# pd3/bcftools

Measured on AMD Instinct MI355X. Metric: variant sites/sec (mpileup|call -m), 1000-sample 30x WGS synthetic, higher is better.
Workload: dtype u8/i32 + f64 likelihood sums

## Files before the change

### bcftools_amd/csrc/api.hip

```cpp
#include <hip/hip_runtime.h>
#include <cstdio>
#include <cstdlib>
#include <cstring>
#include <cmath>
#include <string>
#include <vector>
#include <algorithm>
#include "ctx.h"
#include "tables.h"

using namespace bcfgpu;

static thread_local std::string g_err;
static int set_err(int code, const char *what, hipError_t e = hipSuccess)
{
    char buf[512];
    if (e != hipSuccess) snprintf(buf, sizeof buf, "%s: %s", what, hipGetErrorString(e));
    else snprintf(buf, sizeof buf, "%s", what);
    g_err = buf;
    return code;
}
#define HIPCHK(call) do { hipError_t e_ = (call); if (e_ != hipSuccess) return set_err(BCFGPU_E_HIP, #call, e_); } while (0)

struct bcfgpu_ctx {
// ... 338 lines not shown
    if (!c) return BCFGPU_E_ARG;
    c->timing = on;
    if (on == 2) while (c->pool.size() < 4 * 64) { hipEvent_t e; hipEventCreate(&e); c->pool.push_back(e); }
    return 0;
}
int bcfgpu_timing_get(bcfgpu_ctx *c, bcfgpu_timing *t)
{
    if (!c || !t) return set_err(BCFGPU_E_ARG, "bcfgpu_timing_get: bad arguments");
    if (c->timing == 2) {
        bcfgpu_timing a{};
        const size_t n = c->pool_call.size();
        if (n) {
            HIPCHK(hipStreamSynchronize(c->stream));
            int ncall = 0;
            for (size_t k = 0; k < n; ++k) {
                hipEvent_t *e = &c->pool[4 * k];
                float g = 0, m = 0, q = 0, tot = 0;
                hipEventElapsedTime(&g, e[0], e[1]);
                hipEventElapsedTime(&m, e[1], e[2]);
                if (c->pool_call[k]) { hipEventElapsedTime(&q, e[2], e[3]); hipEventElapsedTime(&tot, e[0], e[3]); ncall++; }
                else hipEventElapsedTime(&tot, e[0], e[2]);
                a.glfgen_ms += g; a.combine_ms += m; a.mcall_ms += q; a.total_ms += tot;
            }
            a.glfgen_ms /= n; a.combine_ms /= n; a.total_ms /= n;
            if (ncall) a.mcall_ms /= ncall;
            c->pool_used = 0; c->pool_call.clear();
        }
        c->last = a;
    }
    *t = c->last;
    return 0;
}

static hipEvent_t *seq_events(bcfgpu_ctx *c)
{
    if (c->timing == 2) {
        while (c->pool.size() < c->pool_used + 4) { hipEvent_t e; hipEventCreate(&e); c->pool.push_back(e); }
        c->pool_call.push_back(0);
        c->pool_used += 4;
        return &c->pool[c->pool_used - 4];
    }
    return c->ev;
}

static int check_tile(bcfgpu_ctx *c, const bcfgpu_tile *t)
{
    if (!t || t->n_sites < 0) return set_err(BCFGPU_E_ARG, "bad tile");
    if (t->n_sites > c->cfg.max_sites || t->n_reads > c->cfg.max_reads)
        return set_err(BCFGPU_E_RANGE, "tile exceeds the capacity the context was created with");
    if (t->n_sites && (!t->plp_off || (!t->is_indel && !t->ref16) || (t->n_reads && (!t->rd || !t->epos))))
        return set_err(BCFGPU_E_ARG, "tile: NULL array");
    if (t->is_indel && t->n_reads && !t->aux) return set_err(BCFGPU_E_ARG, "indel tile without aux");
    if (((uintptr_t)t->rd & 15) || ((uintptr_t)t->epos & 15) || (t->is_indel && ((uintptr_t)t->aux & 15)))
        return set_err(BCFGPU_E_ARG, "tile: rd/epos/aux must be 16-byte aligned");
    if (t->n_reads >> 32) return set_err(BCFGPU_E_RANGE, "tile: more than 2^32-1 reads");
    return 0;
}

static int enqueue_mpileup(bcfgpu_ctx *c, const bcfgpu_tile *tile, const bcfgpu_mplp_out *out)
{
    const int S = c->cfg.n_smpl;
    GlfgenParams g{};
    g.n_sites = tile->n_sites; g.n_smpl = S; g.is_indel = tile->is_indel;
    g.min_baseQ = c->cfg.min_baseQ; g.capQ = c->cfg.capQ; g.fmt_flag = c->cfg.fmt_flag;
    const int slots = 255 / S + 2;
    g.hist_slots = slots <= 8 ? slots : 0;
    {
        const double mean = (double)tile->n_reads / ((double)tile->n_sites * S);
        long want = (long)(mean * 256 * 1.03) + 64;
        want = std::max(2048L, (want + 15) & ~15L);
        int cap = 0;
        for (int wgs = 6; wgs >= 3 && !cap; --wgs) {
            const long budget = (long)(128 / wgs) * 1280 - 32;
            long c = (budget - (long)glfgen_lds_bytes(0, g.hist_slots)) / 2;
            c = std::min(c & ~15L, (long)GLF_MAX_WINDOW);
            if (c >= want || wgs == 3) cap = (int)std::max(c, 2048L);
        }
        g.lds_cap = cap;
        int pc = 64;
        while (pc > 4 && 17 * std::max(g.hist_slots, 1) * pc > 2048) pc >>= 1;
        g.part_cols = pc;
    }
    g.n_reads = (uint32_t)tile->n_reads;
    g.ref16 = tile->ref16; g.off = tile->plp_off; g.rd = tile->rd; g.epos = tile->epos; g.aux = tile->aux;
    g.fk = c->d_fk; g.beta = c->d_beta; g.lhet = c->d_lhet; g.pfx = c->d_pfx;
    g.crp = c->d_crp;
    g.hist = c->d_hist; g.err = c->d_err; g.site_sums = c->d_site_sums;
    g.trunc = reinterpret_cast<unsigned int*>(c->d_err + 1);
    g.deep_list = c->d_deep_list; g.deep_ctr = reinterpret_cast<uint32_t*>(c->d_err + 2); g.deep_keys = c->d_deep_keys;
    g.deep_cap = c->deep_cap; g.deep_key_cap = c->deep_key_cap;
    {
        const int kind = tile->is_indel ? 1 : 0;
        g.draw_bits = (c->draw.rd[kind] && c->draw.rd[kind] == tile->rd && c->draw.n_reads[kind] == tile->n_reads) ? c->draw.bits[kind] : nullptr;
        c->draw.rd[kind] = nullptr;
    }
    g.wide_ctr = reinterpret_cast<uint32_t*>(c->d_err + 5); g.wide_cap = c->wide_cap;
    HIPCHK(hipMemsetAsync(c->d_err + 2, 0, 4 * sizeof(int), c->stream));
    HIPCHK(hipMemsetAsync(c->d_hist, 0, (size_t)tile->n_sites * H_SIZE * sizeof(int), c->stream));
    HIPCHK(hipMemsetAsync(c->d_site_sums, 0, (size_t)tile->n_sites * SITE_NSUM * 8, c->stream));
    hipEvent_t *ev = c->timing ? seq_events(c) : nullptr;
    if (ev) hipEventRecord(ev[0], c->stream);
    launch_glfgen(g, c->stream);
    if (ev) hipEventRecord(ev[1], c->stream);
    CombineParams k{};
    k.n_sites = tile->n_sites; k.n_smpl = S; k.is_indel = tile->is_indel; k.fmt_flag = c->cfg.fmt_flag;
    k.ref16 = tile->ref16; k.cr = c->cr; k.hist = c->d_hist; k.site_sums = c->d_site_sums; k.mw = c->d_mw; k.out = *out;
    launch_combine(k, c->stream);
    if (ev) hipEventRecord(ev[2], c->stream);
    HIPCHK(hipGetLastError());
    return 0;
}

static void finish_timing(bcfgpu_ctx *c, bool with_call)
{
    if (c->timing != 1) return;
    hipEventSynchronize(with_call ? c->ev[3] : c->ev[2]);
    bcfgpu_timing t{};
    hipEventElapsedTime(&t.glfgen_ms, c->ev[0], c->ev[1]);
    hipEventElapsedTime(&t.combine_ms, c->ev[1], c->ev[2]);
    if (with_call) hipEventElapsedTime(&t.mcall_ms, c->ev[2], c->ev[3]);
    hipEventElapsedTime(&t.total_ms, c->ev[0], with_call ? c->ev[3] : c->ev[2]);
    c->last = t;
}

int bcfgpu_mpileup(bcfgpu_ctx *c, const bcfgpu_tile *tile, const bcfgpu_mplp_out *out)
{
    if (!c || !out || !out->site || !out->pl || !out->dp4) return set_err(BCFGPU_E_ARG, "bcfgpu_mpileup: bad arguments");
    int rc = check_tile(c, tile);
    if (rc) return rc;
    if (tile->n_sites == 0) return 0;
    hipSetDevice(c->cfg.device);
    rc = enqueue_mpileup(c, tile, out);
    if (rc) return rc;
    finish_timing(c, false);
    return 0;
}

static float *grp_q_for(bcfgpu_ctx *c, int n_sites)
{
    if (c->cfg.n_grp <= 1 || n_sites <= 0) return nullptr;
    const size_t bytes = (size_t)n_sites * c->cfg.n_grp * 5 * sizeof(float);
    if (bytes <= c->grp_q_bytes) return c->d_grp_q;
    if (c->d_grp_q) { hipStreamSynchronize(c->stream); hipFree(c->d_grp_q); c->d_grp_q = nullptr; c->grp_q_bytes = 0; }
    void *p = nullptr;
    if (hipMalloc(&p, bytes + bytes / 4) != hipSuccess) { (void)hipGetLastError(); return nullptr; }
    c->d_grp_q = (float*)p; c->grp_q_bytes = bytes + bytes / 4;
    return c->d_grp_q;
}

int bcfgpu_mcall(bcfgpu_ctx *c, const bcfgpu_call_in *in, const bcfgpu_call_out *out)
{
    if (!c || !in || !out || !out->site || !out->gt) return set_err(BCFGPU_E_ARG, "bcfgpu_mcall: bad arguments");
    if (in->n_sites == 0) return 0;
    if (!in->nals || !in->unseen || !in->pl || (!in->qs && !(c->cfg.n_grp > 1)))
        return set_err(BCFGPU_E_ARG, "bcfgpu_mcall: NULL input array");
    if (c->cfg.n_grp > 1 && (!in->grp || !in->ad)) return set_err(BCFGPU_E_ARG, "bcfgpu_mcall: -G needs grp and ad");
    if (in->n_gt_max < 1 || in->n_gt_max > BCFGPU_MAX_PL) return set_err(BCFGPU_E_ARG, "bcfgpu_mcall: n_gt_max out of range");
    if (in->ad && (in->n_al_max < 1 || in->n_al_max > BCFGPU_MAX_ALLELES)) return set_err(BCFGPU_E_ARG, "bcfgpu_mcall: n_al_max out of range");
    hipSetDevice(c->cfg.device);
    McallParams m{};
    m.n_sites = in->n_sites; m.n_smpl = c->cfg.n_smpl; m.n_gt_max = in->n_gt_max; m.n_al_max = in->n_al_max;
    m.pl_is_u8 = 0; m.call_flag = c->cfg.call_flag; m.output_tags = c->cfg.output_tags; m.n_grp = c->cfg.n_grp;
    m.theta = c->call_theta_log; m.pl2p = c->d_pl2p;
    m.nals = in->nals; m.unseen = in->unseen; m.msite = nullptr; m.pl = in->pl; m.qs = in->qs; m.ad = in->ad;
    m.grp_rng = c->d_grp_rng; m.grp_q = grp_q_for(c, m.n_sites);
    if (c->cfg.n_grp > 1 && !m.grp_q) return set_err(BCFGPU_E_NOMEM, "call -G: workspace of the groups' frequency sums");
// ... 143 lines not shown
```

### bcftools_amd/csrc/glfgen.hip

```cpp
#include <hip/hip_runtime.h>
#include <cstdlib>
#include "kernels.h"

namespace bcfgpu {

#define WG 256
#ifndef GLF_WAVES
#define GLF_WAVES 5
#endif
#define DEF_MAPQ 20
#define CAP_DIST 25

#define NT16_INT_TBL 0x4444444344424104ull
__device__ __forceinline__ int nt16_int(int c) { return (int)((NT16_INT_TBL >> (4 * (c & 15))) & 7); }
__device__ __forceinline__ int tri(int j, int k) { return k * (k + 1) / 2 + j; }

__device__ __forceinline__ uint32_t wave_sum_u32(uint32_t v)
{
    #pragma unroll
    for (int o = 32; o > 0; o >>= 1) v += __shfl_xor(v, o);
    return v;
}

#define LDS_FK   0
#define LDS_CNT  2112
#ifndef NRANK
#define NRANK 10
#endif
#define NSLOT    NRANK
#ifndef FU
#define FU       4
#endif
#define LDS_HIST_OFF (LDS_CNT + NSLOT * WG * 4)
#define HP_SIZE 280
#define HP_MQS  220
#define HP_MAX  0xffffu
static_assert(GLF_MAX_WINDOW <= HP_MAX, "one round's window alone must fit a 16-bit half of the packed histograms");
static_assert(H_SIZE <= 2 * HP_SIZE, "a deep cell's 32-bit histograms take the LDS of two packed slots (hist_slots >= 2 whenever it is not 0)");
#define NPART 17
static_assert(NPART == SITE_NSUM + 3, "phase A's partial sums: the site totals and three mapQ >= 59 counts");

#define KEY_PACK(rev, q, b, sc) ((uint32_t)(rev) | (uint32_t)(q) << 1 | (uint32_t)(b) << 7 | (uint32_t)(sc) << 10)
#define KEY_REV(k)  ((k) & 1u)
#define KEY_Q(k)    (((k) >> 1) & 63u)
#define KEY_B(k)    (((k) >> 7) & 7u)
#define KEY_SC(k)   (((k) >> 10) & 1u)
#define KEY_PRIM    0x800u

#ifndef WR
#define WR 2
#endif
struct PrimSrc {
    const uint16_t *kpp;
    __device__ __forceinline__ uint32_t key(int j) const { return kpp[j]; }
    __device__ __forceinline__ bool ok(uint32_t k) const { return k != 0; }
    __device__ __forceinline__ int operator()(int j) const { const uint32_t k = key(j); return ok(k) ? (int)(k & 0x7f) : -1; }
};
struct BaseSrc {
    const uint16_t *kp; int b;
    __device__ __forceinline__ uint32_t key(int i) const { return kp[i]; }
    __device__ __forceinline__ bool ok(uint32_t k) const { return KEY_B(k) == (uint32_t)b; }
    __device__ __forceinline__ int operator()(int i) const { const uint32_t k = key(i); return ok(k) ? (int)(k & 0x7f) : -1; }
};
__device__ __forceinline__ uint32_t popc64(uint64_t x) { return (uint32_t)__popc((uint32_t)x) + (uint32_t)__popc((uint32_t)(x >> 32)); }
template <bool FIRST, bool CHK, class Src>
__device__ __forceinline__ void count_keys(uint32_t *s_slot, uint64_t qm, int tid, Src src, int nsrc)
{
    const uint64_t qm1 = qm >> 1;
    for (int j = 0; __any(j < nsrc); j += FU) {
        if (j < nsrc) {
            uint32_t k4[FU];
            #pragma unroll
            for (int u = 0; u < FU; ++u) k4[u] = src.key(j + u);
            #pragma unroll
            for (int u = 0; u < FU; ++u) {
                const uint32_t k = k4[u], q = KEY_Q(k);
                const uint32_t r = popc64(qm1 >> q);
                bool take = src.ok(k) && (u == 0 || j + u < nsrc);
                if (!FIRST) take = take && ((qm >> q) & 1ull);
                if (CHK) take = take && r < (uint32_t)NRANK;
                const uint32_t rv = (uint32_t)((int32_t)(k << 31) >> 31);
                if (take) atomicAdd(&s_slot[r * WG + tid], (rv & 1u) | (~rv & 0x100u));
            }
        }
    }
}
template <bool FIRST, class Src>
__device__ __forceinline__ uint32_t count_runs(uint32_t *s_slot, uint64_t qm, int tid, Src src, int nsrc)
{
    #pragma unroll
    for (int k = 0; k < NRANK; ++k) s_slot[k * WG + tid] = 0;
    if (__any(popc64(qm) > (uint32_t)NRANK)) count_keys<FIRST, true>(s_slot, qm, tid, src, nsrc);
    else count_keys<FIRST, false>(s_slot, qm, tid, src, nsrc);
    uint32_t qs = 0;
    uint64_t m = qm;
    #pragma unroll
    for (int r = 0; r < NRANK && __any(m != 0); ++r) {
        if (m != 0) {
            const uint32_t q = 63u - (uint32_t)__builtin_clzll(m);
            const uint32_t c = s_slot[r * WG + tid];
            s_slot[r * WG + tid] = c | q << 16;
            qs = __builtin_amdgcn_udot4(c, q | q << 8, qs, false);
            m &= ~(1ull << q);
        }
    }
    return qs;
}

template <class Src>
__device__ __forceinline__ double walk_runs(uint32_t *s_slot, uint64_t qm, const double *s_fk, const char *bbase, const double *pfx, int tid,
                                            uint32_t brow, Src src, int nsrc, uint32_t &rev_out, uint32_t &qs_out)
{
    double bs = 0;
    uint32_t qs = 0;
    uint32_t wpack = 0;
    uint32_t cnt = 0;
    uint32_t koff = brow;
    uint32_t qoff = 0;
    uint32_t r = 0;
    uint32_t d_nx = 0;
    auto slot_of = [&](uint32_t rk) -> uint32_t { return s_slot[min(rk, (uint32_t)NRANK - 1u) * WG + tid]; };
    auto step = [&](uint32_t (&off)[WR], uint32_t (&wi)[WR]) -> bool {
        const bool pop = cnt == 0 && r < NRANK;
        cnt = pop ? (d_nx & 0xffu) | (d_nx & 0xff00u) << 8 : cnt;
        qoff = pop ? (d_nx & 0x3f0000u) << 3 : qoff;
        r += pop ? 1u : 0u;
        d_nx = slot_of(r);
        const uint32_t sh = (cnt & 0xffffu) ? 0u : 16u;
        const uint32_t left = (cnt >> sh) & 0xffffu;
        const uint32_t w = (wpack >> sh) & 0xffffu;
        const uint32_t o1 = qoff + koff;
        #pragma unroll
        for (uint32_t u = 0; u < WR; ++u) {
            const bool act = left > u;
            wi[u] = act ? w + u : 256u;
            off[u] = act ? o1 + (u << 11) : brow;
        }
        const uint32_t took = min(left, (uint32_t)WR);
        wpack += took << sh; cnt -= took << sh;
        koff += took << 11;
        return __any(left != 0);
    };
    #define WALK_LOAD(B, F, off_, wi_) do { _Pragma("unroll") for (int u_ = 0; u_ < WR; ++u_) { \
        B[u_] = *reinterpret_cast<const double*>(bbase + (off_)[u_]); F[u_] = s_fk[(wi_)[u_]]; } } while (0)
    #define WALK_ADD(B, F) do { _Pragma("unroll") for (int u_ = 0; u_ < WR; ++u_) bs += F[u_] * B[u_]; } while (0)
    bool first = true;
    while (__any(qm != 0)) {
        qs += first ? count_runs<true>(s_slot, qm, tid, src, nsrc) : count_runs<false>(s_slot, qm, tid, src, nsrc);
        r = 0;
        d_nx = slot_of(0);
        const uint32_t d0 = d_nx, r1 = d0 & 0xffu, f1 = (d0 >> 8) & 0xffu;
        const bool tb = first && brow < (uint32_t)GLF_PFX_N << 3 && (d0 & 0xe0e0u) == 0u && (d0 & 0xffffu) != 0u;
        const uint32_t ti = tb ? (d0 & 0x3f0000u) | brow << 7 | r1 << 5 | f1 : 0u;
        const double t0 = pfx[ti];
        wpack = tb ? r1 | f1 << 16 : wpack;
        koff = tb ? brow + ((r1 + f1) << 11) : koff;
        r = tb ? 1u : 0u;
        d_nx = slot_of(r);
        first = false;
        double bx[WR], fx[WR], by[WR], fy[WR];
        uint32_t off[WR], wi[WR];
        bool ax = step(off, wi);
        WALK_LOAD(bx, fx, off, wi);
        bool ay = step(off, wi);
        WALK_LOAD(by, fy, off, wi);
        bs = tb ? t0 : bs;
        while (ax) {
            WALK_ADD(bx, fx);
            ax = step(off, wi);
            WALK_LOAD(bx, fx, off, wi);
            if (!ay) break;
            WALK_ADD(by, fy);
            ay = step(off, wi);
            WALK_LOAD(by, fy, off, wi);
        }
        WALK_ADD(bx, fx);
        WALK_ADD(by, fy);
        if (__any(__popcll(qm) > NRANK)) {
            uint64_t m = qm;
            for (int k = 0; k < NRANK && m; ++k) m &= ~(1ull << (63 - __clzll((long long)m)));
            qm = m;
        } else qm = 0;
    }
    #undef WALK_ADD
    #undef WALK_LOAD
    rev_out = wpack & 0xffffu; qs_out = qs;
    return bs;
}

struct ReadSums {
    uint32_t t_bq, t_bq2, t_mq, t_mq2, t_md, t_md2;
    uint32_t d_bq, d_bq2, d_mq, d_mq2, d_md, d_md2;
    __device__ __forceinline__ void clear() { t_bq = t_bq2 = t_mq = t_mq2 = t_md = t_md2 = d_bq = d_bq2 = d_mq = d_mq2 = d_md = d_md2 = 0; }
};
struct ReadCounts {
    uint32_t ori, mq0, m59, ref59, rev59;
    __device__ __forceinline__ void clear() { ori = mq0 = m59 = ref59 = rev59 = 0; }
};
typedef unsigned short v2u16 __attribute__((ext_vector_type(2)));

__device__ __forceinline__ uint32_t perm(uint32_t hi, uint32_t lo, uint32_t sel) { return __builtin_amdgcn_perm(hi, lo, sel); }
#define SEL_EVEN 0x0c020c00u
#define SEL_ODD  0x0c030c01u
#define SEL_JOIN 0x06020400u
#define SEL_GE8  0x07030501u
__device__ __forceinline__ v2u16 as_v2(uint32_t x) { return __builtin_bit_cast(v2u16, x); }
__device__ __forceinline__ uint32_t as_u(v2u16 x) { return __builtin_bit_cast(uint32_t, x); }
__device__ __forceinline__ uint32_t pk_min(uint32_t a, uint32_t b) { return as_u(__builtin_elementwise_min(as_v2(a), as_v2(b))); }
__device__ __forceinline__ uint32_t pk_max(uint32_t a, uint32_t b) { return as_u(__builtin_elementwise_max(as_v2(a), as_v2(b))); }
__device__ __forceinline__ uint32_t nonzero80(uint32_t x) { return (((x & 0x7f7f7f7fu) + 0x7f7f7f7fu) | x) & 0x80808080u; }
__device__ __forceinline__ uint32_t bytes_of80(uint32_t m) { return m | (m - (m >> 7)); }
__device__ __forceinline__ uint32_t byte_at(uint32_t x, int u) { return (x >> (8 * u)) & 0xffu; }

template <bool INDEL, bool LDS_HIST, bool DEEP>
__global__ __launch_bounds__(WG) __attribute__((amdgpu_waves_per_eu(GLF_WAVES, GLF_WAVES))) void glfgen_kernel(const GlfgenParams P)
{
    extern __shared__ __align__(16) unsigned char smem[];
    if (DEEP && (blockIdx.x >= P.deep_ctr[0] || P.deep_list[2 * blockIdx.x] == 0xffffffffu)) return;
    const int cap = DEEP ? 0x7ffffff0 : P.lds_cap;
    double   *s_fk  = reinterpret_cast<double*>(smem + LDS_FK);
    uint32_t *s_cnt = reinterpret_cast<uint32_t*>(smem + LDS_CNT);
    int      *s_hist = reinterpret_cast<int*>(smem + LDS_HIST_OFF);
    unsigned long long *s_tot = reinterpret_cast<unsigned long long*>(s_hist + (size_t)P.hist_slots * HP_SIZE);
    uint32_t *s_part = s_cnt;
    const int pcol = P.part_cols;
    uint16_t *s_key = DEEP ? P.deep_keys + P.deep_list[2 * blockIdx.x + 1]
                           : reinterpret_cast<uint16_t*>(s_tot + (size_t)P.hist_slots * SITE_NSUM);
    __shared__ unsigned int s_next, s_skip, s_pend;
    constexpr bool PACKED = LDS_HIST && !DEEP;

    const int tid = threadIdx.x;
    const int S = P.n_smpl;
    const long ncells = (long)P.n_sites * S;
    const long cell0 = DEEP ? (long)P.deep_list[2 * blockIdx.x] : (long)blockIdx.x * WG;
    const long cell_end = DEEP ? cell0 + 1 : min(cell0 + WG, ncells);
    const int site0 = (int)(cell0 / S);
    const int site_last = (int)((cell_end - 1) / S);

    const long cell = cell0 + tid;
    const bool active = cell < cell_end;

    s_fk[tid] = P.fk[tid];
    if (tid < 8) s_fk[256 + tid] = 0.0;
    if (LDS_HIST) {
        for (int i = tid; i < P.hist_slots * HP_SIZE; i += WG) s_hist[i] = 0;
        for (int i = tid; i < P.hist_slots * SITE_NSUM; i += WG) s_tot[i] = 0;
    }

    int site = 0, ref4c = 4;
    uint32_t beg = 0, end = 0;
    if (active) {
        site = (int)(cell / S);
        beg = P.off[cell]; end = P.off[cell + 1];
        if (!INDEL) ref4c = nt16_int(P.ref16[site]);
    }
    const int primary = INDEL ? 0 : ref4c;
    uint32_t fmt_flag = (uint32_t)P.fmt_flag;
    asm volatile("" : "+s"(fmt_flag));
    const bool want_epos = (fmt_flag & (BCFGPU_INFO_RPB | BCFGPU_INFO_VDB)) != 0;
    const bool want_scr = (fmt_flag & (BCFGPU_INFO_SCR | BCFGPU_FMT_SCR)) != 0;
    const uint32_t span_end = P.off[cell_end];
    uint32_t n_reads_tot = P.n_reads, min_baseQ = (uint32_t)P.min_baseQ, capQ = (uint32_t)P.capQ;
    asm volatile("" : "+s"(n_reads_tot), "+s"(min_baseQ), "+s"(capQ));
    const uint32_t *p_rd = P.rd, *p_aux = P.aux, *p_off = P.off;
    const uint8_t *p_epos = P.epos;
    asm volatile("" : "+s"(p_rd), "+s"(p_aux), "+s"(p_off), "+s"(p_epos));

    bool done = !active;
    bool deep = false;
    if (!DEEP && active && end - beg > (uint32_t)cap - 3u) {
        deep = true;
        const uint32_t need = (end - beg + 16u) & ~7u;
        const uint32_t slot = atomicAdd(&P.deep_ctr[0], 1u), at = atomicAdd(&P.deep_ctr[1], need);
        const bool room = at + need <= P.deep_key_cap;
        if (slot < P.deep_cap) { P.deep_list[2 * slot] = room ? (uint32_t)cell : 0xffffffffu; P.deep_list[2 * slot + 1] = room ? at : 0u; }
        if (slot >= P.deep_cap || !room) { atomicExch(P.err, BCFGPU_E_DEPTH); atomicExch(&P.deep_ctr[2], 1u); }
    }
    uint32_t base = p_off[cell0];
    if (PACKED && tid == 0) s_pend = min((base & ~3u) + (uint32_t)cap, span_end) - base;

    auto flush_packed = [&](const bool clear) {
        const int nslot = min(P.hist_slots, P.n_sites - site0);
        for (int i = tid; i < nslot * HP_SIZE; i += WG) {
            const uint32_t v = (uint32_t)s_hist[i];
            if (!v) continue;
            if (clear) s_hist[i] = 0;
            const int sl = i / HP_SIZE, j = i - sl * HP_SIZE;
            int *g = P.hist + (long)(site0 + sl) * H_SIZE;
            const int lo = j < HP_MQS ? j : H_FWD_MQS + (j - HP_MQS), hi = j < HP_MQS ? j + H_ALT_OFF : H_REV_MQS + (j - HP_MQS);
            if (v & 0xffffu) atomicAdd(&g[lo], (int)(v & 0xffffu));
            if (v >> 16) atomicAdd(&g[hi], (int)(v >> 16));
        }
    };

    for (;;) {
        const uint32_t abase = base & ~3u;
        const uint32_t lim = DEEP ? span_end : min(abase + (uint32_t)cap, span_end);
        if (tid == 0) { s_next = 0xffffffffu; s_skip = 0; }
        if (LDS_HIST) {
            int i0 = tid;
            asm volatile("" : "+v"(i0));
            for (int i = i0; i < P.hist_slots * NPART * pcol; i += WG) s_part[i] = 0;
        }
        __syncthreads();
        const bool cand = !done && !deep && beg >= base && end <= lim;
        if (!done && !cand) atomicMin(&s_next, beg);
        __syncthreads();
        const uint32_t nb = s_next;
        const uint32_t rlim = min(nb, lim);
        const bool part = cand && end <= rlim;

        for (int sg = site0; sg <= site_last; ++sg) {
            const long c_lo = max(cell0, (long)sg * S), c_hi = min(cell_end, (long)(sg + 1) * S);
            const uint32_t rb = max(p_off[c_lo], base), re = min(p_off[c_hi], rlim);
            if (rb >= re) continue;
            const int ref_base = INDEL ? -1 : (int)P.ref16[sg];
            const uint32_t ref4 = INDEL ? 4u : (uint32_t)nt16_int(ref_base);
            const uint32_t primq = INDEL ? 0u : ref4;
            const unsigned long long tbl = (NT16_INT_TBL & ~0xfull) | (unsigned long long)ref4;
            int *hist = LDS_HIST ? s_hist + (sg - site0) * HP_SIZE : P.hist + (long)sg * H_SIZE;
            ReadSums A; A.clear();
            ReadCounts C; C.clear();
            const uint32_t tlo_lo = 0x04010000u | ref4, tlo_hi = 0x04040402u, thi_lo = 0x04040403u, thi_hi = 0x04040404u;
            const uint32_t kq = 0x01000100u - min(min_baseQ, 256u) * 0x00010001u;
            const uint32_t cap2 = min(capQ, 0xffffu) * 0x00010001u;
            const uint32_t refb4 = (uint32_t)(ref_base & 15) * 0x01010101u, prim4 = primq * 0x01010101u;
            const uint32_t scm = want_scr ? 0x04040404u : 0u;
            const bool all_diff = !INDEL && ref4 >= 4;
            const bool no_ref = INDEL || ref_base < 0 || ref_base > 15;

            auto quad = [&](const uint4 &w4, const uint4 &a4, uint32_t e4, uint32_t vm4, uint32_t &k01, uint32_t &k23) {
                const uint32_t t0 = perm(w4.y, w4.x, 0x05010400u), t1 = perm(w4.y, w4.x, 0x07030602u);
                const uint32_t t2 = perm(w4.w, w4.z, 0x05010400u), t3 = perm(w4.w, w4.z, 0x07030602u);
                uint32_t B4 = perm(t2, t0, 0x05040100u);
                const uint32_t M4 = perm(t2, t0, 0x07060302u);
                const uint32_t F4 = (vm4 & perm(t3, t1, 0x05040100u)) | (~vm4 & 0x80808080u);
                const uint32_t D4 = perm(t3, t1, 0x07060302u);
                uint32_t QR4, BB4;
                uint32_t ok80;
// ... 41 lines not shown
                const uint32_t khi = (((BB4 >> 1) & 0x03030303u) | ((F4 >> 3) & scm) | ((nprim80 ^ 0x80808080u) >> 4)) & OK4;
                k01 = perm(khi, klo, 0x05010400u); k23 = perm(khi, klo, 0x07030602u);
                const uint32_t Bm = B4 & OK4, Mm = Mf4 & OK4, Dm = Df4 & OK4;
                A.t_bq = __builtin_amdgcn_udot4(Bm, 0x01010101u, A.t_bq, false); A.t_bq2 = __builtin_amdgcn_udot4(Bm, Bm, A.t_bq2, false);
                A.t_mq = __builtin_amdgcn_udot4(Mm, 0x01010101u, A.t_mq, false); A.t_mq2 = __builtin_amdgcn_udot4(Mm, Mm, A.t_mq2, false);
                A.t_md = __builtin_amdgcn_udot4(Dm, 0x01010101u, A.t_md, false); A.t_md2 = __builtin_amdgcn_udot4(Dm, Dm, A.t_md2, false);
                const uint32_t dif80 = ok80 & (all_diff ? 0x80808080u : nprim80);
                if (dif80) {
                    const uint32_t DM = bytes_of80(dif80);
                    const uint32_t bd = Bm & DM, qd = Mm & DM, dd = Dm & DM;
                    A.d_bq = __builtin_amdgcn_udot4(bd, 0x01010101u, A.d_bq, false); A.d_bq2 = __builtin_amdgcn_udot4(bd, bd, A.d_bq2, false);
                    A.d_mq = __builtin_amdgcn_udot4(qd, 0x01010101u, A.d_mq, false); A.d_mq2 = __builtin_amdgcn_udot4(qd, qd, A.d_mq2, false);
                    A.d_md = __builtin_amdgcn_udot4(dd, 0x01010101u, A.d_md, false); A.d_md2 = __builtin_amdgcn_udot4(dd, dd, A.d_md2, false);
                }
                #pragma unroll
                for (int u = 0; u < 4; ++u) {
                    if (!((ok80 >> (8 * u + 7)) & 1)) continue;
                    const bool isref = !((nref80 >> (8 * u + 7)) & 1), rev = (F4 >> (8 * u + 4)) & 1;
                    const uint32_t bq = byte_at(B4, u), mapQ = byte_at(Mf4, u), pos = byte_at(e4, u);
                    const bool m59 = (m59_80 >> (8 * u + 7)) & 1;
                    if (PACKED) {
                        const int inc = isref ? 1 : 0x10000;
                        atomicAdd(&hist[H_REF_POS + pos], inc);
                        atomicAdd(&hist[H_REF_BQ + min(bq, 59u)], inc);
                        if (!m59) {
                            atomicAdd(&hist[H_REF_MQ + mapQ], inc);
                            atomicAdd(&hist[HP_MQS + mapQ], rev ? 0x10000 : 1);
                        }
                    } else {
                        const uint32_t aoff = isref ? 0u : (uint32_t)H_ALT_OFF;
                        atomicAdd(&hist[aoff + H_REF_POS + pos], 1);
                        atomicAdd(&hist[aoff + H_REF_BQ + min(bq, 59u)], 1);
                        if (!m59) {
                            atomicAdd(&hist[aoff + H_REF_MQ + mapQ], 1);
                            atomicAdd(&hist[(rev ? H_REV_MQS : H_FWD_MQS) + mapQ], 1);
                        }
                    }
                }
            };

            const uint32_t g0 = rb & ~3u;
            uint4 w4n = make_uint4(0, 0, 0, 0), a4n = make_uint4(0, 0, 0, 0);
            uint32_t e4n = 0;
            auto fetch = [&](uint32_t i4) {
                if (i4 >= re) return;
                if (i4 + 3 < n_reads_tot) {
                    w4n = *reinterpret_cast<const uint4*>(p_rd + i4);
                    if (want_epos) e4n = *reinterpret_cast<const uint32_t*>(p_epos + i4);
                    if (INDEL) a4n = *reinterpret_cast<const uint4*>(p_aux + i4);
                } else {
                    uint32_t t4[4] = {0, 0, 0, 0}, x4[4] = {0, 0, 0, 0};
                    e4n = 0;
                    for (int j = 0; j < 4; ++j) if (i4 + j < n_reads_tot) {
                        t4[j] = p_rd[i4 + j];
                        if (want_epos) e4n |= (uint32_t)p_epos[i4 + j] << (8 * j);
                        if (INDEL) x4[j] = p_aux[i4 + j];
                    }
                    w4n = make_uint4(t4[0], t4[1], t4[2], t4[3]); a4n = make_uint4(x4[0], x4[1], x4[2], x4[3]);
                }
            };
            fetch(g0 + 4u * tid);
            for (uint32_t i4 = g0 + 4u * tid; i4 < re; i4 += 4u * WG) {
                const uint4 w4 = w4n, a4 = a4n;
                const uint32_t e4 = e4n;
                fetch(i4 + 4u * WG);
                const uint32_t lo = rb > i4 ? rb - i4 : 0u, hi = min(re - i4, 4u);
                const uint32_t vm4 = (0xffffffffu << (8 * lo)) & (hi == 4u ? 0xffffffffu : ~(0xffffffffu << (8 * hi)));
                uint32_t k01, k23;
                quad(w4, a4, e4, vm4, k01, k23);
                const uint32_t ko = i4 - abase;
                if (vm4 == 0xffffffffu) {
                    *reinterpret_cast<uint2*>(s_key + ko) = make_uint2(k01, k23);
                } else {
                    const uint32_t kv[4] = { k01 & 0xffffu, k01 >> 16, k23 & 0xffffu, k23 >> 16 };
                    #pragma unroll
                    for (int u = 0; u < 4; ++u) if ((vm4 >> (8 * u)) & 1) s_key[ko + u] = (uint16_t)kv[u];
                }
            }
            const uint32_t v[NPART] = { A.t_bq - A.d_bq, A.t_bq2 - A.d_bq2, A.d_bq, A.d_bq2, A.t_mq - A.d_mq, A.t_mq2 - A.d_mq2, A.d_mq, A.d_mq2,
                                        A.t_md - A.d_md, A.t_md2 - A.d_md2, A.d_md, A.d_md2, C.ori, C.mq0, C.m59, C.ref59, C.rev59 };
            if (LDS_HIST) {
                int col = tid & (pcol - 1);
                asm volatile("" : "+v"(col));
                uint32_t *pt = s_part + (sg - site0) * (NPART * pcol) + col;
                #pragma unroll
                for (int j = 0; j < NPART; ++j) atomicAdd(&pt[j * pcol], v[j]);
            } else {
                unsigned long long *tot = P.site_sums + (size_t)sg * SITE_NSUM;
                uint32_t x[NPART];
                #pragma unroll
                for (int j = 0; j < NPART; ++j) x[j] = wave_sum_u32(v[j]);
                if ((tid & 63) == 0) {
                    #pragma unroll
                    for (int j = 0; j < SITE_NSUM; ++j) if (x[j]) atomicAdd(&tot[j], (unsigned long long)x[j]);
                    const uint32_t m59 = x[SITE_NSUM], ref59 = x[SITE_NSUM + 1], rev59 = x[SITE_NSUM + 2];
                    if (ref59) atomicAdd(&hist[H_REF_MQ + 59], (int)ref59);
                    if (m59 - ref59) atomicAdd(&hist[H_ALT_MQ + 59], (int)(m59 - ref59));
                    if (m59 - rev59) atomicAdd(&hist[H_FWD_MQS + 59], (int)(m59 - rev59));
                    if (rev59) atomicAdd(&hist[H_REV_MQS + 59], (int)rev59);
                }
            }
        }
        __syncthreads();
        if (LDS_HIST) {
            const int nslot = min(P.hist_slots, P.n_sites - site0), q4 = pcol >> 2;
            int i0 = tid;
            asm volatile("" : "+v"(i0));
            for (int i = i0; i < nslot * NPART * 4; i += WG) {
                const uint32_t *pt = s_part + (i >> 2) * pcol + (i & 3) * q4;
                unsigned long long x = 0;
                for (int k = 0; k < q4; ++k) x += pt[k];
                x += __shfl_xor(x, 1); x += __shfl_xor(x, 2);
                if ((i & 3) == 0 && x) {
                    const int vi = i >> 2, sl = vi / NPART, j = vi % NPART;
                    if (j < SITE_NSUM) s_tot[sl * SITE_NSUM + j] += x;
                    else {
                        const int c = (int)(uint32_t)x;
                        int *g = P.hist + (long)(site0 + sl) * H_SIZE;
                        if (j == SITE_NSUM) { atomicAdd(&g[H_ALT_MQ + 59], c); atomicAdd(&g[H_FWD_MQS + 59], c); }
                        else if (j == SITE_NSUM + 1) { atomicAdd(&g[H_REF_MQ + 59], c); atomicAdd(&g[H_ALT_MQ + 59], -c); }
                        else { atomicAdd(&g[H_REV_MQS + 59], c); atomicAdd(&g[H_FWD_MQS + 59], -c); }
                    }
                }
            }
            __syncthreads();
        }

        uint16_t *kp_w = s_key + (part ? beg - abase : 0);
        const uint16_t *kp = kp_w;
        const int cnt_raw = part ? (int)(end - beg) : 0;
        if (__any(cnt_raw > BCFGPU_MAX_DEPTH)) {
            if (cnt_raw > BCFGPU_MAX_DEPTH) {
                uint32_t nus = 0;
                for (int i = 0; i < cnt_raw; ++i) nus += kp_w[i] != 0 ? 1u : 0u;
                const volatile unsigned long long *t = reinterpret_cast<const volatile unsigned long long*>(P.crp);
                uint64_t *qs64_p = reinterpret_cast<uint64_t*>(t[2]); uint32_t *misc_p = reinterpret_cast<uint32_t*>(t[6]);
                uint32_t mark = 0;
                if (nus > BCFGPU_MAX_DEPTH) {
                    uint32_t qs[4] = {0, 0, 0, 0}, af[4] = {0, 0, 0, 0}, ar[4] = {0, 0, 0, 0}, cn[4] = {0, 0, 0, 0}, sc = 0, acc = 0;
                    const bool all_diff = !INDEL && ref4c >= 4;
                    bool planned = false;
                    if (P.draw_bits) {
                        uint32_t nm = 0;
                        for (int i = 0; i < cnt_raw; ++i) { const uint32_t ri = beg + (uint32_t)i; nm += (kp_w[i] != 0 && ((P.draw_bits[ri >> 5] >> (ri & 31)) & 1u)) ? 1u : 0u; }
                        planned = nm == BCFGPU_MAX_DEPTH;
                    }
                    for (int i = 0; i < cnt_raw; ++i) {
                        const uint32_t k = kp_w[i];
                        if (k == 0) continue;
                        const uint32_t rev = KEY_REV(k), q = KEY_Q(k), b = KEY_B(k);
                        const uint32_t dr = ((all_diff || !(k & KEY_PRIM)) ? 2u : 0u) | rev;
                        #pragma unroll
                        for (uint32_t x = 0; x < 4; ++x) {
                            qs[x] += b == x ? q : 0u;
                            af[x] += (b == x && !rev) ? 1u : 0u; ar[x] += (b == x && rev) ? 1u : 0u;
                            cn[x] += dr == x ? 1u : 0u;
                        }
                        sc += KEY_SC(k);
                        bool stays = ++acc <= BCFGPU_MAX_DEPTH;
                        if (planned) { const uint32_t ri = beg + (uint32_t)i; stays = ((P.draw_bits[ri >> 5] >> (ri & 31)) & 1u) != 0; }
                        if (!stays) kp_w[i] = 0;
                    }
                    const uint32_t slot = atomicAdd(P.wide_ctr, 1u);
                    const uint32_t big = af[0] | af[1] | af[2] | af[3] | ar[0] | ar[1] | ar[2] | ar[3] | cn[0] | cn[1] | cn[2] | cn[3] | sc;
                    if (slot >= P.wide_cap || big > 0xffffu) atomicExch(P.err, BCFGPU_E_DEPTH);
                    else {
                        WideRec *w = reinterpret_cast<WideRec*>(t[7]) + slot;
                        #pragma unroll
                        for (int x = 0; x < 4; ++x) { w->qs[x] = qs[x]; w->ad[x] = af[x] | ar[x] << 16; }
                        w->cnt[0] = cn[0] | cn[1] << 16; w->cnt[1] = cn[2] | cn[3] << 16;
                        w->scr = sc; w->n = nus; w->cell = (uint32_t)cell; w->pad[0] = w->pad[1] = w->pad[2] = 0;
                        qs64_p[cell] = WIDE_QS_MARK | slot;
                        mark = CR_WIDE;
                    }
                    if (!planned) atomicAdd(P.trunc, 1u);
                }
                misc_p[cell] = mark;
            }
        }
        uint32_t scr = 0;
        if (want_scr) for (int i = 0; i < cnt_raw; ++i) scr += KEY_SC((uint32_t)kp[i]);
        uint64_t qmask = 0;
        uint32_t n_prim = 0;
        uint64_t qs64 = 0;
        uint64_t ad64 = 0;
        uint32_t n_b4 = 0;
        uint32_t o_rev = 0, n_other = 0;
        {
            uint32_t k_nx = kp[0];
            for (int i = 0; i < cnt_raw; ++i) {
                const uint32_t k = k_nx;
                k_nx = kp[i + 1];
                const uint32_t pb = k >> 11;
                qmask |= (uint64_t)pb << KEY_Q(k);
                n_prim += pb;
                if (k - 1u < KEY_PRIM - 1u) {
                    const uint32_t t = kp_w[n_other], rev = KEY_REV(k), q = KEY_Q(k), b = KEY_B(k);
                    kp_w[n_other] = (uint16_t)k; kp_w[i] = (uint16_t)t;
                    ++n_other; o_rev += rev;
                    if (b < 4) { qs64 += (uint64_t)q << (16 * b); ad64 += 1ull << (8 * b + 32 * rev); }
                    else ++n_b4;
                }
            }
        }
        const uint32_t n = n_prim + n_other;
        const bool dead_cell = n == 0;
        const char *bbase = reinterpret_cast<const char*>(P.beta);
        const uint32_t brow = n << 3;

        double bsum[5] = {0, 0, 0, 0, 0};
        uint32_t prim_rev = 0, qs_prim = 0;
        {
            const uint16_t *kpp = kp + n_other;
            const PrimSrc psrc{kpp};
            const double bs = walk_runs(s_cnt, qmask, s_fk, bbase, P.pfx, tid, brow, psrc, dead_cell ? 0 : cnt_raw - (int)n_other, prim_rev, qs_prim);
            #pragma unroll
            for (int b = 0; b < 5; ++b) if (b == primary) bsum[b] = bs;
        }
        if (primary < 4) {
            qs64 += (uint64_t)qs_prim << (16 * primary);
            ad64 += (uint64_t)(n_prim - prim_rev) << (8 * primary) | (uint64_t)prim_rev << (8 * primary + 32);
        } else n_b4 += n_prim;
        int c[5];
        #pragma unroll
        for (int b = 0; b < 4; ++b) c[b] = (int)((ad64 >> (8 * b)) & 0xff) + (int)((ad64 >> (8 * b + 32)) & 0xff);
        c[4] = (int)n_b4;
        if (__any(n_other > 0)) {
            #pragma unroll 1
            for (int b = 0; b < 5; ++b) {
                int cb = b == 0 ? c[0] : b == 1 ? c[1] : b == 2 ? c[2] : b == 3 ? c[3] : c[4];
                if (b == primary || dead_cell) cb = 0;
                if (!__any(cb > 0)) continue;
                const BaseSrc src{kp, b};
                const int no = cb > 0 ? (int)n_other : 0;
                double bs;
                if (!__any(cb > 1)) {
                    int key = -1;
                    for (int i = 0; __any(i < no); ++i) { const int k7 = i < no ? src(i) : -1; if (k7 >= 0) key = k7; }
                    const uint32_t off1 = key >= 0 ? ((uint32_t)(key >> 1) << 19) + brow : brow;
                    const double B1 = *reinterpret_cast<const double*>(bbase + off1);
                    const double F1 = key >= 0 ? s_fk[0] : s_fk[256];
                    bs = 0.;
                    bs += F1 * B1;
                } else {
                uint64_t qm = 0;
                for (int i = 0; i < no; ++i) { const int key = src(i); if (key >= 0) qm |= 1ull << (key >> 1); }
                uint32_t r_, q_;
                bs = walk_runs(s_cnt, qm, s_fk, bbase, P.pfx, tid, brow, src, no, r_, q_);
                }
                if (cb > 0) {
                    #pragma unroll
                    for (int bb = 0; bb < 5; ++bb) if (bb == b) bsum[bb] = bs;
                }
            }
        }
        const uint32_t n_rev = prim_rev + o_rev;

        uint32_t code = 0;
        CallretPlanes cr;
        {
            const volatile unsigned long long *t = reinterpret_cast<const volatile unsigned long long*>(P.crp);
            cr.p15 = reinterpret_cast<float*>(t[0]); cr.pa = reinterpret_cast<float*>(t[1]);
            cr.qs64 = reinterpret_cast<uint64_t*>(t[2]); cr.adf = reinterpret_cast<uint32_t*>(t[3]);
            cr.adr = reinterpret_cast<uint32_t*>(t[4]); cr.cnt4 = reinterpret_cast<uint32_t*>(t[5]);
            cr.misc = reinterpret_cast<uint32_t*>(t[6]);
        }
        if (part) {
            const int nbases = (c[0] > 0) + (c[1] > 0) + (c[2] > 0) + (c[3] > 0) + (c[4] > 0);
            if (nbases <= 1) {
                const int b = c[1] > 0 ? 1 : c[2] > 0 ? 2 : c[3] > 0 ? 3 : c[4] > 0 ? 4 : 0;
                double bsb = bsum[0];
                #pragma unroll
                for (int k = 1; k < 5; ++k) if (k == b) bsb = bsum[k];
                float A = n > 0 ? (float)((double)0.0f + bsb) : 0.0f;
                if (A < 0.0f) A = 0.0f;
                cr.pa[cell] = A;
                code = (uint32_t)b;
            } else {
                code = CR_FULL;
                float *p15c = cr.p15 + (size_t)cell * 16;
                #pragma unroll
                for (int j = 0; j < 5; ++j) {
                    float tmp1 = 0.0f; int tmp2 = 0;
                    #pragma unroll
                    for (int k = 0; k < 5; ++k) { if (k == j) continue; tmp1 = (float)((double)tmp1 + bsum[k]); tmp2 += c[k]; }
                    float v = 0.0f;
                    if (n > 0 && tmp2) v = tmp1;
                    if (v < 0.0f) v = 0.0f;
                    p15c[tri(j, j)] = v;
                    #pragma unroll
                    for (int k = j + 1; k < 5; ++k) {
                        const int cjk = c[j] + c[k];
                        float t1 = 0.0f; int t2 = 0;
                        #pragma unroll
                        for (int i = 0; i < 5; ++i) { if (i == j || i == k) continue; t1 = (float)((double)t1 + bsum[i]); t2 += c[i]; }
                        float h = 0.0f;
                        if (n > 0) {
                            const double lh = -4.343 * P.lhet[cjk << 8 | c[k]];
                            h = t2 ? (float)(lh + (double)t1) : (float)lh;
                            if (h < 0.0f) h = 0.0f;
                        }
                        p15c[tri(j, k)] = h;
                    }
                }
            }
        }
        if (part) {
            const bool all_diff = (!INDEL && ref4c >= 4);
            const uint32_t n_fwd = n - n_rev;
            const uint32_t d_rev = all_diff ? n_rev : o_rev, d_fwd = all_diff ? n_fwd : n_other - o_rev;
            const uint32_t cnt4 = (n_fwd - d_fwd) | (n_rev - d_rev) << 8 | d_fwd << 16 | d_rev << 24;
            uint32_t wm = 0;
            if (cnt_raw > BCFGPU_MAX_DEPTH) wm = *reinterpret_cast<volatile uint32_t*>(&cr.misc[cell]) & CR_WIDE;
            if (!wm) cr.qs64[cell] = qs64;
            cr.adf[cell] = (uint32_t)ad64; cr.adr[cell] = (uint32_t)(ad64 >> 32); cr.cnt4[cell] = cnt4;
            cr.misc[cell] = code | wm | (scr & 0xff) << 8;
            done = true;
        }
        if (nb == 0xffffffffu) break;
        base = nb;
        if (!DEEP && !done && deep && beg == base) s_skip = end;
        __syncthreads();
        if (!DEEP) {
            const uint32_t sk = s_skip, pend = PACKED ? s_pend : 0u;
            if (sk) { if (deep && beg == base) done = true; base = sk; }
            __syncthreads();
            if (PACKED) {
                const uint32_t win = min((base & ~3u) + (uint32_t)cap, span_end) - base, p = pend + win;
                const bool fl = p > HP_MAX;
                if (tid == 0) s_pend = fl ? win : p;
                if (fl) flush_packed(true);
            }
        }
    }

    if (LDS_HIST) {
        __syncthreads();
        const int nslot = min(P.hist_slots, P.n_sites - site0);
        if (PACKED) flush_packed(false);
        else {
            int *g = P.hist + (long)site0 * H_SIZE;
            for (int i = tid; i < H_SIZE; i += WG) { const int v = s_hist[i]; if (v) atomicAdd(&g[i], v); }
        }
        for (int i = tid; i < nslot * SITE_NSUM; i += WG) {
            const unsigned long long v = s_tot[i];
            if (v) atomicAdd(&P.site_sums[(size_t)site0 * SITE_NSUM + i], v);
        }
    }
}

static_assert(2 * GLF_PFX_S - 3 < 256 && GLF_PFX_N <= 256 && GLF_PFX_S <= 256, "the prefix table stays inside fk[256] and beta[64][256][256]");
__global__ __launch_bounds__(WG) void glfgen_prefix_kernel(const double *fk, const double *beta, double *pfx)
{
    const uint32_t i = blockIdx.x * WG + threadIdx.x;
    if (i >= 64u * GLF_PFX_S * GLF_PFX_N) return;
    const uint32_t n = i % GLF_PFX_N, r = i / GLF_PFX_N % GLF_PFX_S, q = i / (GLF_PFX_N * GLF_PFX_S);
    const double *b = beta + ((size_t)q << 16 | n);
    double *t = pfx + (((size_t)q * GLF_PFX_N + n) * GLF_PFX_S + r) * GLF_PFX_S;
    double bs = 0;
    for (uint32_t u = 0; u < r; ++u) bs += fk[u] * b[u << 8];
    t[0] = bs;
    for (uint32_t u = 0; u + 1 < (uint32_t)GLF_PFX_S; ++u) { bs += fk[u] * b[(r + u) << 8]; t[u + 1] = bs; }
}

void launch_glfgen_prefix(const double *fk, const double *beta, double *pfx, hipStream_t s)
{
    hipLaunchKernelGGL(glfgen_prefix_kernel, dim3(64 * GLF_PFX_S * GLF_PFX_N / WG), dim3(WG), 0, s, fk, beta, pfx);
}

size_t glfgen_lds_bytes(int cap, int hist_slots)
{
    return LDS_HIST_OFF + (size_t)hist_slots * (HP_SIZE * sizeof(int) + SITE_NSUM * 8) + ((size_t)cap + 8) * 2;
}

template <bool INDEL, bool LDS_HIST>
static void launch_one(const GlfgenParams &p, hipStream_t s, int grid, size_t lds)
{
    if (lds > 48 * 1024)
        hipFuncSetAttribute(reinterpret_cast<const void*>(glfgen_kernel<INDEL, LDS_HIST, false>),
                            hipFuncAttributeMaxDynamicSharedMemorySize, (int)lds);
    hipLaunchKernelGGL((glfgen_kernel<INDEL, LDS_HIST, false>), dim3(grid), dim3(WG), lds, s, p);
    if (p.deep_cap) hipLaunchKernelGGL((glfgen_kernel<INDEL, LDS_HIST, true>), dim3(p.deep_cap), dim3(WG), glfgen_lds_bytes(0, p.hist_slots), s, p);
}

void launch_glfgen(const GlfgenParams &p, hipStream_t s)
{
    const long ncells = (long)p.n_sites * p.n_smpl;
    if (ncells == 0) return;
    const int grid = (int)((ncells + WG - 1) / WG);
    const size_t lds = glfgen_lds_bytes(p.lds_cap, p.hist_slots);
    if (p.is_indel) { if (p.hist_slots) launch_one<true, true>(p, s, grid, lds); else launch_one<true, false>(p, s, grid, lds); }
    else            { if (p.hist_slots) launch_one<false, true>(p, s, grid, lds); else launch_one<false, false>(p, s, grid, lds); }
}

}
```

### bcftools_amd/csrc/kernels.h

```cpp
#pragma once
#include <hip/hip_runtime.h>
#include <vector>
#include <stdint.h>
#include "../../include/bcfgpu.h"

namespace bcfgpu {

enum : int {
    H_REF_POS = 0, H_REF_MQ = 100, H_REF_BQ = 160, H_ALT_OFF = 220,
    H_ALT_POS = H_REF_POS + H_ALT_OFF, H_ALT_MQ = H_REF_MQ + H_ALT_OFF, H_ALT_BQ = H_REF_BQ + H_ALT_OFF,
    H_FWD_MQS = 440, H_REV_MQS = 500, H_SIZE = 560
};
enum : int { SITE_NSUM = 14 };
enum : int { GLF_MAX_WINDOW = 16384 };
enum : int { GLF_PFX_N = 64, GLF_PFX_S = 32 };
enum : size_t { GLF_PFX_DOUBLES = (size_t)64 * GLF_PFX_N * GLF_PFX_S * GLF_PFX_S };

struct CallretPlanes {
    float    *p15;
    float    *pa;
    uint64_t *qs64;
    uint32_t *adf;
    uint32_t *adr;
    uint32_t *cnt4;
    uint32_t *misc;
    struct WideRec *wide;
};

enum : uint32_t { CR_FULL = 0x80, CR_WIDE = 0x40 };
#define WIDE_QS_MARK (0xffffull << 48)

struct WideRec {
    uint32_t qs[4];
    uint32_t ad[4];
    uint32_t cnt[2];
    uint32_t scr, n;
    uint32_t cell, pad[3];
};
static_assert(sizeof(WideRec) == 64, "one cache-line-aligned record per over-deep cell");

struct GlfgenParams {
    int n_sites, n_smpl, is_indel;
    int min_baseQ, capQ, fmt_flag;
    int hist_slots;
    int lds_cap;
    int part_cols;
    uint32_t n_reads;
    const int8_t   *ref16;
    const uint32_t *off;
    const uint32_t *rd;
    const uint8_t  *epos;
    const uint32_t *aux;
    const double *fk, *beta, *lhet;
    const double *pfx;
    const CallretPlanes *crp;
    int *hist;
    unsigned long long *site_sums;
    int *err;
    unsigned int *trunc;
    uint32_t *wide_ctr;
    const uint32_t *draw_bits;
    uint32_t wide_cap;
    uint32_t *deep_list;
    uint32_t *deep_ctr;
    uint16_t *deep_keys;
    uint32_t deep_cap, deep_key_cap;
};

struct DrawState {
    uint64_t x = 0x1234ABCD330EULL;
    const uint32_t *rd[2] = {nullptr, nullptr};
    uint64_t n_reads[2] = {0, 0};
    uint32_t *bits[2] = {nullptr, nullptr};
    uint32_t n_planned = 0;
};

struct CombineParams {
    int n_sites, n_smpl, is_indel, fmt_flag;
    const int8_t *ref16;
    CallretPlanes cr;
    const int *hist;
    const unsigned long long *site_sums;
    const double *mw;
    int vec4;
    bcfgpu_mplp_out out;
};

struct McallParams {
    int n_sites, n_smpl;
    int n_gt_max, n_al_max;
    int pl_is_u8;
    int call_flag, output_tags, n_grp;
    double theta;
    const double *pl2p;
    const int32_t *nals, *unseen;
    const bcfgpu_site *msite;
    const void *pl;
    const float *qs;
    const int32_t *ad;
    const uint16_t *ad_u16, *ad_u16b; const int32_t *qs_i32;
    const uint8_t *ploidy;
    const int32_t *grp;
    int32_t *grp_rng;
    float *grp_q;
    const int32_t *prior_an, *prior_ac;
    const float *i16;
    bcfgpu_call_out out;
    int out_n_gt_max;
    int *err;
    int small_too;
};

struct DevPool {
    int valid, n_reads;
    uint32_t n_bases, n_cig;
    const int32_t *r_pos, *r_lq, *r_flag, *r_ncig, *r_cig_off, *r_seq_off;
    uint8_t *r_mapq;
    const uint32_t *cig;
    const uint8_t *seq16;
    uint8_t *qual;
    uint8_t *zq, *r_has_zq;
    uint8_t *keep;
    int ext_valid, ext_lo, ext_hi;
    int qual_slot;
};

struct ReadMeta;
struct PileupParams {
    int n_sites, n_smpl, beg, want_epos, max_span;
    const int32_t *smpl_off;
// ... 99 lines not shown
```

Baseline: 6.512 million.

## Cut register and ALU cost in glfgen with packed counts and fast site division

Several micro-optimizations land in the glfgen kernel together. Run-count packing changes so the reverse and forward counts sit in the low bytes of each 16-bit half and the quality moves to bits 8-13, which simplifies the unpacking in walk_runs. The 64-bit cell/S division is replaced by a host-precomputed 20-bit reciprocal multiply when indices fit in 32 bits, and LDS histogram clearing uses 16-byte stores. Inline-asm register constraints steer values into scalar or vector registers to reduce register pressure. The risks are that the reciprocal shortcut could be exact only within the bounded remainder range and that counts are now limited to 8 bits per half.

```diff
diff --git a/bcftools_amd/csrc/api.hip b/bcftools_amd/csrc/api.hip
--- a/bcftools_amd/csrc/api.hip
+++ b/bcftools_amd/csrc/api.hip
@@ -444,6 +444,8 @@
         g.part_cols = pc;
     }
     g.n_reads = (uint32_t)tile->n_reads;
+    g.site_mul = (long)tile->n_sites * S < (1L << 31) ? (uint32_t)(((1L << 20) + S - 1) / S) : 0u;
+    if (getenv("BCFGPU_INDEX64")) g.site_mul = 0;
     g.ref16 = tile->ref16; g.off = tile->plp_off; g.rd = tile->rd; g.epos = tile->epos; g.aux = tile->aux;
     g.fk = c->d_fk; g.beta = c->d_beta; g.lhet = c->d_lhet; g.pfx = c->d_pfx;
     g.crp = c->d_crp;
diff --git a/bcftools_amd/csrc/glfgen.hip b/bcftools_amd/csrc/glfgen.hip
--- a/bcftools_amd/csrc/glfgen.hip
+++ b/bcftools_amd/csrc/glfgen.hip
@@ -80,7 +80,7 @@
                 if (!FIRST) take = take && ((qm >> q) & 1ull);
                 if (CHK) take = take && r < (uint32_t)NRANK;
                 const uint32_t rv = (uint32_t)((int32_t)(k << 31) >> 31);
-                if (take) atomicAdd(&s_slot[r * WG + tid], (rv & 1u) | (~rv & 0x100u));
+                if (take) atomicAdd(&s_slot[r * WG + tid], (rv & 1u) | (~rv & 0x10000u));
             }
         }
     }
@@ -99,8 +99,8 @@
         if (m != 0) {
             const uint32_t q = 63u - (uint32_t)__builtin_clzll(m);
             const uint32_t c = s_slot[r * WG + tid];
-            s_slot[r * WG + tid] = c | q << 16;
-            qs = __builtin_amdgcn_udot4(c, q | q << 8, qs, false);
+            s_slot[r * WG + tid] = c | q << 8;
+            qs = __builtin_amdgcn_udot4(c, q | q << 16, qs, false);
             m &= ~(1ull << q);
         }
     }
@@ -122,8 +122,8 @@
     auto slot_of = [&](uint32_t rk) -> uint32_t { return s_slot[min(rk, (uint32_t)NRANK - 1u) * WG + tid]; };
     auto step = [&](uint32_t (&off)[WR], uint32_t (&wi)[WR]) -> bool {
         const bool pop = cnt == 0 && r < NRANK;
-        cnt = pop ? (d_nx & 0xffu) | (d_nx & 0xff00u) << 8 : cnt;
-        qoff = pop ? (d_nx & 0x3f0000u) << 3 : qoff;
+        cnt = pop ? d_nx & 0x00ff00ffu : cnt;
+        qoff = pop ? (d_nx & 0x3f00u) << 11 : qoff;
         r += pop ? 1u : 0u;
         d_nx = slot_of(r);
         const uint32_t sh = (cnt & 0xffffu) ? 0u : 16u;
@@ -133,8 +133,10 @@
         #pragma unroll
         for (uint32_t u = 0; u < WR; ++u) {
             const bool act = left > u;
-            wi[u] = act ? w + u : 256u;
-            off[u] = act ? o1 + (u << 11) : brow;
+            uint32_t wu = act ? w : 256u - u, ou = act ? o1 : brow;
+            if (u) asm("" : "+v"(wu));
+            wi[u] = wu + u;
+            off[u] = ou;
         }
         const uint32_t took = min(left, (uint32_t)WR);
         wpack += took << sh; cnt -= took << sh;
@@ -142,18 +144,18 @@
         return __any(left != 0);
     };
     #define WALK_LOAD(B, F, off_, wi_) do { _Pragma("unroll") for (int u_ = 0; u_ < WR; ++u_) { \
-        B[u_] = *reinterpret_cast<const double*>(bbase + (off_)[u_]); F[u_] = s_fk[(wi_)[u_]]; } } while (0)
+        B[u_] = *reinterpret_cast<const double*>(bbase + (off_)[u_] + ((size_t)u_ << 11)); F[u_] = s_fk[(wi_)[u_]]; } } while (0)
     #define WALK_ADD(B, F) do { _Pragma("unroll") for (int u_ = 0; u_ < WR; ++u_) bs += F[u_] * B[u_]; } while (0)
     bool first = true;
     while (__any(qm != 0)) {
         qs += first ? count_runs<true>(s_slot, qm, tid, src, nsrc) : count_runs<false>(s_slot, qm, tid, src, nsrc);
         r = 0;
         d_nx = slot_of(0);
-        const uint32_t d0 = d_nx, r1 = d0 & 0xffu, f1 = (d0 >> 8) & 0xffu;
-        const bool tb = first && brow < (uint32_t)GLF_PFX_N << 3 && (d0 & 0xe0e0u) == 0u && (d0 & 0xffffu) != 0u;
-        const uint32_t ti = tb ? (d0 & 0x3f0000u) | brow << 7 | r1 << 5 | f1 : 0u;
+        const uint32_t d0 = d_nx, r1 = d0 & 0xffu, f1 = (d0 >> 16) & 0xffu;
+        const bool tb = first && brow < (uint32_t)GLF_PFX_N << 3 && (d0 & 0x00e000e0u) == 0u && (d0 & 0x00ff00ffu) != 0u;
+        const uint32_t ti = tb ? (d0 & 0x3f00u) << 8 | brow << 7 | r1 << 5 | f1 : 0u;
         const double t0 = pfx[ti];
-        wpack = tb ? r1 | f1 << 16 : wpack;
+        wpack = tb ? d0 & 0x00ff00ffu : wpack;
         koff = tb ? brow + ((r1 + f1) << 11) : koff;
         r = tb ? 1u : 0u;
         d_nx = slot_of(r);
@@ -234,27 +236,37 @@
     const long ncells = (long)P.n_sites * S;
     const long cell0 = DEEP ? (long)P.deep_list[2 * blockIdx.x] : (long)blockIdx.x * WG;
     const long cell_end = DEEP ? cell0 + 1 : min(cell0 + WG, ncells);
-    const int site0 = (int)(cell0 / S);
-    const int site_last = (int)((cell_end - 1) / S);
-
     const long cell = cell0 + tid;
     const bool active = cell < cell_end;
+    int site0, site_last, site = 0;
+    if (P.site_mul) {
+        const uint32_t S32 = (uint32_t)S, c0 = (uint32_t)cell0, s0 = c0 / S32, rem0 = c0 - s0 * S32;
+        const uint32_t mul = P.site_mul;
+        auto quot = [&](uint32_t x) -> uint32_t { return S32 >= (uint32_t)WG ? (x >= S32 ? 1u : 0u) : (x * mul) >> 20; };
+        site0 = (int)s0;
+        site_last = (int)(s0 + quot(rem0 + (uint32_t)(cell_end - 1 - cell0)));
+        site = (int)(s0 + quot(rem0 + (uint32_t)tid));
+    } else {
+        site0 = (int)(cell0 / S);
+        site_last = (int)((cell_end - 1) / S);
+        if (active) site = (int)(cell / S);
+    }
 
     s_fk[tid] = P.fk[tid];
     if (tid < 8) s_fk[256 + tid] = 0.0;
     if (LDS_HIST) {
-        for (int i = tid; i < P.hist_slots * HP_SIZE; i += WG) s_hist[i] = 0;
-        for (int i = tid; i < P.hist_slots * SITE_NSUM; i += WG) s_tot[i] = 0;
-    }
-
-    int site = 0, ref4c = 4;
+        static_assert(LDS_HIST_OFF % 16 == 0 && (HP_SIZE * 4 + SITE_NSUM * 8) % 16 == 0, "the slots' LDS is cleared 16 bytes at a time");
+        uint4 *z = reinterpret_cast<uint4*>(s_hist);
+        for (int i = tid; i < P.hist_slots * ((HP_SIZE * 4 + SITE_NSUM * 8) / 16); i += WG) z[i] = make_uint4(0, 0, 0, 0);
+    }
+
+    int ref4c = 4;
     uint32_t beg = 0, end = 0;
     if (active) {
-        site = (int)(cell / S);
         beg = P.off[cell]; end = P.off[cell + 1];
         if (!INDEL) ref4c = nt16_int(P.ref16[site]);
     }
-    const int primary = INDEL ? 0 : ref4c;
+    const int primary_cell = INDEL ? 0 : ref4c;
     uint32_t fmt_flag = (uint32_t)P.fmt_flag;
     asm volatile("" : "+s"(fmt_flag));
     const bool want_epos = (fmt_flag & (BCFGPU_INFO_RPB | BCFGPU_INFO_VDB)) != 0;
@@ -462,9 +474,11 @@
             if (LDS_HIST) {
                 int col = tid & (pcol - 1);
                 asm volatile("" : "+v"(col));
-                uint32_t *pt = s_part + (sg - site0) * (NPART * pcol) + col;
+                int pc = pcol;
+                asm volatile("" : "+s"(pc));
+                uint32_t *pt = s_part + (sg - site0) * (NPART * pc) + col;
                 #pragma unroll
-                for (int j = 0; j < NPART; ++j) atomicAdd(&pt[j * pcol], v[j]);
+                for (int j = 0; j < NPART; ++j) atomicAdd(&pt[j * pc], v[j]);
             } else {
                 unsigned long long *tot = P.site_sums + (size_t)sg * SITE_NSUM;
                 uint32_t x[NPART];
@@ -483,11 +497,11 @@
         }
         __syncthreads();
         if (LDS_HIST) {
-            const int nslot = min(P.hist_slots, P.n_sites - site0), q4 = pcol >> 2;
-            int i0 = tid;
-            asm volatile("" : "+v"(i0));
+            int i0 = tid, hs = P.hist_slots, pc = pcol;
+            asm volatile("" : "+v"(i0), "+s"(hs), "+s"(pc));
+            const int nslot = min(hs, P.n_sites - site0), q4 = pc >> 2;
             for (int i = i0; i < nslot * NPART * 4; i += WG) {
-                const uint32_t *pt = s_part + (i >> 2) * pcol + (i & 3) * q4;
+                const uint32_t *pt = s_part + (i >> 2) * pc + (i & 3) * q4;
                 unsigned long long x = 0;
                 for (int k = 0; k < q4; ++k) x += pt[k];
                 x += __shfl_xor(x, 1); x += __shfl_xor(x, 2);
@@ -506,6 +520,9 @@
             __syncthreads();
         }
 
+        int tid_b = tid;
+        if (INDEL) asm volatile("" : "+v"(tid_b));
+        const long cell_b = cell0 + tid_b;
         uint16_t *kp_w = s_key + (part ? beg - abase : 0);
         const uint16_t *kp = kp_w;
         const int cnt_raw = part ? (int)(end - beg) : 0;
@@ -549,13 +566,13 @@
                         #pragma unroll
                         for (int x = 0; x < 4; ++x) { w->qs[x] = qs[x]; w->ad[x] = af[x] | ar[x] << 16; }
                         w->cnt[0] = cn[0] | cn[1] << 16; w->cnt[1] = cn[2] | cn[3] << 16;
-                        w->scr = sc; w->n = nus; w->cell = (uint32_t)cell; w->pad[0] = w->pad[1] = w->pad[2] = 0;
-                        qs64_p[cell] = WIDE_QS_MARK | slot;
+                        w->scr = sc; w->n = nus; w->cell = (uint32_t)cell_b; w->pad[0] = w->pad[1] = w->pad[2] = 0;
+                        qs64_p[cell_b] = WIDE_QS_MARK | slot;
                         mark = CR_WIDE;
                     }
                     if (!planned) atomicAdd(P.trunc, 1u);
                 }
-                misc_p[cell] = mark;
+                misc_p[cell_b] = mark;
             }
         }
         uint32_t scr = 0;
@@ -590,6 +607,8 @@
 
         double bsum[5] = {0, 0, 0, 0, 0};
         uint32_t prim_rev = 0, qs_prim = 0;
+        int primary = primary_cell;
+        if (!INDEL) asm volatile("" : "+v"(primary));
         {
             const uint16_t *kpp = kp + n_other;
             const PrimSrc psrc{kpp};
@@ -654,11 +673,11 @@
                 for (int k = 1; k < 5; ++k) if (k == b) bsb = bsum[k];
                 float A = n > 0 ? (float)((double)0.0f + bsb) : 0.0f;
                 if (A < 0.0f) A = 0.0f;
-                cr.pa[cell] = A;
+                cr.pa[cell_b] = A;
                 code = (uint32_t)b;
             } else {
                 code = CR_FULL;
-                float *p15c = cr.p15 + (size_t)cell * 16;
+                float *p15c = cr.p15 + (size_t)cell_b * 16;
                 #pragma unroll
                 for (int j = 0; j < 5; ++j) {
                     float tmp1 = 0.0f; int tmp2 = 0;
@@ -686,15 +705,15 @@
             }
         }
         if (part) {
-            const bool all_diff = (!INDEL && ref4c >= 4);
+            const bool all_diff = (!INDEL && primary >= 4);
             const uint32_t n_fwd = n - n_rev;
             const uint32_t d_rev = all_diff ? n_rev : o_rev, d_fwd = all_diff ? n_fwd : n_other - o_rev;
             const uint32_t cnt4 = (n_fwd - d_fwd) | (n_rev - d_rev) << 8 | d_fwd << 16 | d_rev << 24;
             uint32_t wm = 0;
-            if (cnt_raw > BCFGPU_MAX_DEPTH) wm = *reinterpret_cast<volatile uint32_t*>(&cr.misc[cell]) & CR_WIDE;
-            if (!wm) cr.qs64[cell] = qs64;
-            cr.adf[cell] = (uint32_t)ad64; cr.adr[cell] = (uint32_t)(ad64 >> 32); cr.cnt4[cell] = cnt4;
-            cr.misc[cell] = code | wm | (scr & 0xff) << 8;
+            if (cnt_raw > BCFGPU_MAX_DEPTH) wm = *reinterpret_cast<volatile uint32_t*>(&cr.misc[cell_b]) & CR_WIDE;
+            if (!wm) cr.qs64[cell_b] = qs64;
+            cr.adf[cell_b] = (uint32_t)ad64; cr.adr[cell_b] = (uint32_t)(ad64 >> 32); cr.cnt4[cell_b] = cnt4;
+            cr.misc[cell_b] = code | wm | (scr & 0xff) << 8;
             done = true;
         }
         if (nb == 0xffffffffu) break;
diff --git a/bcftools_amd/csrc/kernels.h b/bcftools_amd/csrc/kernels.h
--- a/bcftools_amd/csrc/kernels.h
+++ b/bcftools_amd/csrc/kernels.h
@@ -46,6 +46,7 @@
     int lds_cap;
     int part_cols;
     uint32_t n_reads;
+    uint32_t site_mul;
     const int8_t   *ref16;
     const uint32_t *off;
     const uint32_t *rd;
```

After: 6.568 million (median of 6 runs). No clear change (+0.9%).
